# freiberg-roman/mj-grasp-sim

Hardware: NVIDIA B200
Metric: env_steps_per_s (higher is better)
Workload: dtype f32

## Files before the change

mj_grasp_sim_b200/csrc/mgs_common.cuh:

```cuda
#pragma once
#include <math.h>
#include <stdint.h>
#include <string.h>

#ifdef MGS_REAL_DOUBLE
typedef double real;
#define R_(x) x
#define REAL_EPS 2.2e-16
#else
typedef float real;
#define R_(x) x##f
#define REAL_EPS 1.2e-7f
#endif
#define MGS_MINVAL R_(1e-15)
#if !defined(MGS_REAL_DOUBLE) && !defined(MGS_NO_QPOS_COMP)
#define MGS_QPOS_COMP 1
#define MGS_NQ_LO(nq) (nq)
#else
#define MGS_NQ_LO(nq) 0
#endif

#ifdef MGS_HOST
#define MGS_DEV static inline
#define MGS_DEVN static
#define LANES 1
#define MGS_LANE 0
#define WSYNC() ((void)0)
#define LDG(p) (*(p))
#define MGS_STAGE_BARRIER(k) ((void)0)
#elif defined(MGS_WIDE)
#include <cuda_runtime.h>
#define MGS_DEV __device__ __forceinline__
#define MGS_DEVN static __device__ __noinline__
#define LANES MGS_WIDE
#define MGS_LANE ((int)threadIdx.x)
#define WSYNC() __syncthreads()
#define LDG(p) __ldg(p)
#define MGS_STAGE_BARRIER(k) ((void)0)
#else
#include <cuda_runtime.h>
#define MGS_DEV __device__ __forceinline__
#define MGS_DEVN static __device__ __noinline__
#define LANES 32
#define MGS_LANE ((int)(threadIdx.x & 31))
#define WSYNC() __syncwarp()
#define LDG(p) __ldg(p)
#ifndef MGS_BAR_MASK
#define MGS_BAR_MASK 63
#endif
#define MGS_STAGE_BARRIER(k) do { if ((MGS_BAR_MASK >> (k)) & 1) __syncthreads(); } while (0)
#endif

#ifndef MGS_INNER_UNROLL
#define MGS_INNER_UNROLL 4
#endif
#define MGS_PRAGMA_(x) _Pragma(#x)
#define MGS_PRAGMA(x) MGS_PRAGMA_(x)
#define MGS_UNROLL_INNER MGS_PRAGMA(unroll MGS_INNER_UNROLL)

#define PFOR(i, n) for (int i = MGS_LANE; i < (n); i += LANES)

enum { JNT_FREE = 0, JNT_BALL = 1, JNT_SLIDE = 2, JNT_HINGE = 3 };
enum { GEOM_SPHERE = 2, GEOM_CAPSULE = 3, GEOM_CYLINDER = 5, GEOM_BOX = 6, GEOM_MESH = 7 };
enum { EQ_CONNECT = 0, EQ_WELD = 1, EQ_JOINT = 2 };
enum { CT_EQUALITY = 0, CT_FRICTION_DOF = 1, CT_LIMIT = 2, CT_CONTACT = 3 };
enum { ST_SATISFIED = 0, ST_QUADRATIC = 1, ST_LINEARNEG = 2, ST_LINEARPOS = 3, ST_CONE = 4 };
enum { MGS_MODE_STEP = 0, MGS_MODE_COLLISION = 1, MGS_MODE_STABILITY = 2, MGS_MODE_CLUTTER_COLLISION = 3, MGS_MODE_CLUTTER_STABLE = 4 };

struct DevModel {
  int nq, nv, nu, nbody, njnt, neq, nmocap, ntendon, nwrap, ncgeom, npair, nhull;
  int maxdepth, max_tree_dofs, nM, ntree, ne_rows, nf_rows, ngravcomp, dofmask_words, cone_elliptic, iterations, ls_iterations, noslip_iterations, mpr_iterations, ground_geomid;
  real timestep, impratio, tolerance, ls_tolerance, noslip_tolerance, mpr_tolerance, meaninertia, gravity[3];
  const int *body_parentid, *body_rootid, *body_mocapid, *body_jntadr, *body_jntnum, *body_dofadr, *body_dofnum, *body_depth;
  const real *body_pos, *body_quat, *body_ipos, *body_iquat, *body_mass, *body_inertia, *body_invweight0, *body_subtreemass, *body_gravcomp;
  const int *jnt_type, *jnt_bodyid, *jnt_qposadr, *jnt_dofadr, *jnt_limited;
  const real *jnt_pos, *jnt_axis, *jnt_range, *jnt_stiffness, *jnt_solref, *jnt_solimp, *jnt_margin, *qpos0, *qpos_spring;
  const int *dof_bodyid, *dof_jntid, *dof_parentid, *dof_treeadr, *dof_treenum;
  const real *dof_armature, *dof_damping, *dof_frictionloss, *dof_solref, *dof_solimp, *dof_invweight0;
  const int *cgeom_geomid, *cgeom_type, *cgeom_bodyid, *cgeom_hullid;
  const real *cgeom_pos, *cgeom_quat, *cgeom_size, *cgeom_rbound;
  const int *hull_vertadr, *hull_vertnum, *hull_faceadr, *hull_facenum, *hull_facevertadr, *hull_facevertnum, *hull_facevert;
  const int *hull_nbradr, *hull_nbrnum, *hull_nbr;
  const real *hull_vert, *hull_facenormal;
  const int *pair_geom1, *pair_geom2, *pair_condim;
  const real *pair_friction, *pair_solref, *pair_solimp, *pair_margin;
  const int *tendon_adr, *tendon_num, *wrap_dofadr, *wrap_qposadr;
  const real *wrap_coef;
  const int *actuator_trntype, *actuator_trnid, *actuator_ctrllimited, *actuator_forcelimited;
  const real *actuator_gainprm, *actuator_biasprm, *actuator_ctrlrange, *actuator_forcerange, *actuator_gear;
  const int *eq_type, *eq_obj1id, *eq_obj2id, *eq_active, *eq_rowadr, *tri_ab;
  const int *dof_frictionrank;
  const int *dof_rowoff;
  const int *dof_blk;
  const int *blk_ij;
  const int *dof_treeid, *body_treeid;
  const int *tri_madr;
  const unsigned int *body_dofmask;
  const real *eq_data, *eq_solref, *eq_solimp;
  const real *mocap_pos0, *mocap_quat0;
};

#define MGS_LAYOUT_PERSIST(X)                                                                                      \
  X(hdr, 8) X(qpos, nq) X(qpos_lo, MGS_NQ_LO(nq)) X(qvel, nv) X(qacc_ws, nv) X(ctrl, nu) X(mocap, 7 * nmocap)                                          \
  X(xpos, 3 * nbody) X(xquat, 4 * nbody) X(xmat, 9 * nbody) X(rootcom, 3 * nbody) X(cdof, 6 * nv)                  \
  X(M, nM) X(Minv, nM) X(H, nv * nv)                                                                     \
  X(ten_length, ntendon) X(ten_J, ntendon * nv) X(act_moment, nu * nv) X(act_force, nu) X(act_length, nu)          \
  X(qfrc_smooth, nv) X(qacc_smooth, nv) X(qacc, nv) X(qfrc_constraint, nv) X(Ma, nv) X(grad, nv) X(search, nv)     \
  X(Mv, nv) X(wvec, nv) X(con_pos, 3 * ncon_max) X(con_normal, 3 * ncon_max) X(con_dist, ncon_max)                 \
  X(con_mu, ncon_max) X(con_pair, ncon_max) X(con_efc, ncon_max) X(nsB, 3 * nv) X(nsS, lanes + (lanes > 32 ? 8 : 0)) X(mpr_cache, 4 * ncache)
#define MGS_LAYOUT_TRANSIENT(X)                                                                                    \
  X(xipos, 3 * nbody) X(ximat, 9 * nbody) X(xanchor, 3 * njnt) X(xaxis, 3 * njnt) X(gxpos, 3 * ncgeom)             \
  X(gxmat, 9 * ncgeom) X(cinert, 10 * nbody) X(crb, 10 * nbody) X(cdof_dot, 6 * nv) X(cvel, 6 * nbody)             \
  X(cacc, 6 * nbody) X(cfrc, 6 * nbody)
#define MGS_LAYOUT_SOLVER(X)                                                                                       \
  X(J, nefc_max * nv) X(efc_D, nefc_max) X(efc_R, nefc_max) X(efc_aref, nefc_max) X(efc_aux, nefc_max)             \
  X(efc_force, nefc_max) X(efc_jar, nefc_max) X(efc_jv, nefc_max) X(efc_tsi, nefc_max)                                       \
  X(efc_key, (lanes > 32 ? nefc_max : 0)) X(efc_list, (lanes > 32 ? nefc_max : 0))
#define MGS_LAYOUT_FIELDS(X) MGS_LAYOUT_PERSIST(X) MGS_LAYOUT_TRANSIENT(X) MGS_LAYOUT_SOLVER(X)

struct Layout {
#define X(name, cnt) int name;
  MGS_LAYOUT_FIELDS(X)
#undef X
  int total, ncon_max, nefc_max, ncache;
  int req_off;
  int clip_off, nclip;
};

#define MGS_CLIP_STRIDE 109
#define MGS_MPR_CACHE_MAX 128
static inline void layout_compute(Layout *L, int nq, int nv, int nu, int nbody, int njnt, int nmocap, int ntendon, int ncgeom,
                                  int ncon_max, int nefc_max, int npair, int nM, int lanes = 32, int ncache_max = MGS_MPR_CACHE_MAX) {
  int off = 0;
  const int ncache = npair < ncache_max ? npair : ncache_max;
  L->ncache = ncache;
#define X(name, cnt) L->name = off; off += (cnt);
  MGS_LAYOUT_PERSIST(X)
  const int overlay = off;
  MGS_LAYOUT_TRANSIENT(X)
  const int end_t = off;
  off = overlay;
  MGS_LAYOUT_SOLVER(X)
#undef X
  L->total = off > end_t ? off : end_t;
  L->clip_off = end_t;
  L->nclip = (L->total - end_t) / MGS_CLIP_STRIDE;
  if (L->nclip < 1) { L->nclip = 1; L->total = end_t + MGS_CLIP_STRIDE; }
  if (L->nclip > 32) L->nclip = 32;
  L->req_off = L->clip_off + L->nclip * MGS_CLIP_STRIDE;
  if (lanes > 32 && L->total < L->req_off + 6 * lanes) L->total = L->req_off + 6 * lanes;
  L->total = (L->total + 3) & ~3;
  L->ncon_max = ncon_max;
  L->nefc_max = nefc_max;
}

#define MGS_MAX_NU 24
#define MGS_MAX_NJ 24
struct RolloutParams {
  int mode, n, nj, base_qposadr, nstep, nstep_close, nstep_lift, shake_steps, repose_on_close;
  real lift_dist, shake_dist;
  real qvel_clip;
  int joint_qposadr[MGS_MAX_NJ];
  real close_ctrl[MGS_MAX_NU];
};

struct BatchIO {
  const float *pose7;
  const float *joints;
  uint8_t *labels;
  int *steps;
  const real *state_in;
  real *state_out;
  real *diag_out;
  float *aux;
  int state_stride, diag_stride;
  unsigned int *work_counter;
  int *mpr_cache_g;
  real *env_state;
  const int *scene_index;
  int nscene;
  unsigned int *scene_success;
  int enough_stable;
};
```

mj_grasp_sim_b200/csrc/mgs_model_build.h:

```cpp
#pragma once
#include <string>
#include <vector>

#include "../../include/mgs_model_desc.h"
#include "mgs_common.cuh"

struct ModelBlob {
  std::vector<char> bytes;
  DevModel dm;
  int ncon_max, nefc_max;
  int rows_static, rows_per_contact;
  int nfreeobj;
};

namespace mgs_detail {
template <typename T, typename S>
inline const T *put(std::vector<char> &b, const S *src, size_t n) {
  size_t off = (b.size() + 15) & ~size_t(15);
  b.resize(off + (n ? n : 1) * sizeof(T));
  T *dst = reinterpret_cast<T *>(b.data() + off);
  for (size_t i = 0; i < n; i++) dst[i] = (T)src[i];
  return reinterpret_cast<const T *>(off);
}
}

inline bool build_model_blob(const MgsModelDesc *d, ModelBlob &out, std::string &err) {
  using mgs_detail::put;
  DevModel &m = out.dm;
  std::vector<char> &b = out.bytes;
  b.clear();
  b.resize(16);
  memset(&m, 0, sizeof(m));
  if (d->nu > MGS_MAX_NU) { err = "too many actuators"; return false; }
  if (d->nv > 255) { err = "nv > 255 (the lower-triangle index table packs a dof index in 8 bits)"; return false; }
  if (d->nmocap > 1) { err = "at most one mocap body is supported"; return false; }
  for (int p = 0; p < d->npair; p++)
    if (d->pair_condim[p] != 1 && d->pair_condim[p] != 3 && d->pair_condim[p] != 4) { err = "condim must be 1, 3 or 4"; return false; }
  for (int g = 0; g < d->ncgeom; g++) {
    int t = d->cgeom_type[g];
    if (t != GEOM_SPHERE && t != GEOM_CAPSULE && t != GEOM_CYLINDER && t != GEOM_BOX && t != GEOM_MESH) { err = "unsupported geom type"; return false; }
  }
  m.nq = d->nq; m.nv = d->nv; m.nu = d->nu; m.nbody = d->nbody; m.njnt = d->njnt; m.neq = d->neq; m.nmocap = d->nmocap;
  m.ntendon = d->ntendon; m.nwrap = d->nwrap; m.ncgeom = d->ncgeom; m.npair = d->npair; m.nhull = d->nhull;
  m.cone_elliptic = d->cone_elliptic; m.iterations = d->iterations; m.ls_iterations = d->ls_iterations;
  m.noslip_iterations = d->noslip_iterations; m.mpr_iterations = d->mpr_iterations; m.ground_geomid = d->ground_geomid;
  m.timestep = (real)d->timestep; m.impratio = (real)d->impratio; m.tolerance = (real)d->tolerance; m.ls_tolerance = (real)d->ls_tolerance;
  m.noslip_tolerance = (real)d->noslip_tolerance; m.mpr_tolerance = (real)d->mpr_tolerance; m.meaninertia = (real)d->meaninertia;
  for (int k = 0; k < 3; k++) m.gravity[k] = (real)d->gravity[k];
  const int nb = d->nbody, nv = d->nv, nq = d->nq, nj = d->njnt, nu = d->nu, ng = d->ncgeom, np = d->npair, nh = d->nhull;
  std::vector<int> depth(nb, 0), rowadr(d->neq, 0);
  std::vector<double> stm(nb, 0.0);
  int maxdepth = 0;
  for (int i = 1; i < nb; i++) { depth[i] = depth[d->body_parentid[i]] + 1; if (depth[i] > maxdepth) maxdepth = depth[i]; }
  for (int i = 0; i < nb; i++) stm[i] = d->body_mass[i];
  for (int i = nb - 1; i > 0; i--) stm[d->body_parentid[i]] += stm[i];
  int ne = 0;
  for (int q = 0; q < d->neq; q++) {
    rowadr[q] = ne;
    if (d->eq_active[q]) ne += d->eq_type[q] == EQ_WELD ? 6 : (d->eq_type[q] == EQ_CONNECT ? 3 : 1);
  }
  m.maxdepth = maxdepth; m.ne_rows = ne;
#define PI_(f, n) m.f = put<int>(b, d->f, (size_t)(n))
#define PR_(f, n) m.f = put<real>(b, d->f, (size_t)(n))
  PI_(body_parentid, nb); PI_(body_rootid, nb); PI_(body_mocapid, nb); PI_(body_jntadr, nb); PI_(body_jntnum, nb); PI_(body_dofadr, nb);
  PI_(body_dofnum, nb);
  m.body_depth = put<int>(b, depth.data(), nb);
  PR_(body_pos, 3 * nb); PR_(body_quat, 4 * nb); PR_(body_ipos, 3 * nb); PR_(body_iquat, 4 * nb); PR_(body_mass, nb); PR_(body_inertia, 3 * nb);
  PR_(body_invweight0, 2 * nb);
  m.body_subtreemass = put<real>(b, stm.data(), nb);
  PR_(body_gravcomp, nb);
  for (int i = 0; i < nb; i++) m.ngravcomp += (d->body_gravcomp[i] != 0 && d->body_mass[i] != 0);
  PI_(jnt_type, nj); PI_(jnt_bodyid, nj); PI_(jnt_qposadr, nj); PI_(jnt_dofadr, nj); PI_(jnt_limited, nj);
  PR_(jnt_pos, 3 * nj); PR_(jnt_axis, 3 * nj); PR_(jnt_range, 2 * nj); PR_(jnt_stiffness, nj); PR_(jnt_solref, 2 * nj); PR_(jnt_solimp, 5 * nj);
  PR_(jnt_margin, nj); PR_(qpos0, nq); PR_(qpos_spring, nq);
  PI_(dof_bodyid, nv); PI_(dof_jntid, nv); PI_(dof_parentid, nv);
  {
    std::vector<int> tadr(nv, 0), tnum(nv, 0);
    int maxt = 0;
    for (int i = 0; i < nv;) {
      int root = d->body_rootid[d->dof_bodyid[i]], j = i;
      while (j < nv && d->body_rootid[d->dof_bodyid[j]] == root) j++;
      for (int k = i; k < j; k++) { tadr[k] = i; tnum[k] = j - i; }
      if (j - i > maxt) maxt = j - i;
      i = j;
    }
    m.dof_treeadr = put<int>(b, tadr.data(), nv);
    m.dof_treenum = put<int>(b, tnum.data(), nv);
    m.max_tree_dofs = maxt;
    std::vector<int> rowoff(nv > 0 ? nv : 1, 0), ij;
    int nM = 0;
    for (int i = 0; i < nv;) {
      const int t = tnum[i];
      for (int r = 0; r < t; r++) {
        rowoff[i + r] = nM + r * t - i;
        for (int c = 0; c < t; c++) ij.push_back(((i + r) << 8) | (i + c));
      }
      nM += t * t;
      i += t;
    }
    m.nM = nM;
    std::vector<int> dtree(nv > 0 ? nv : 1, 0), btree(nb, -1);
    int ntree = 0;
    for (int i = 0; i < nv;) { for (int k = 0; k < tnum[i]; k++) dtree[i + k] = ntree; ntree++; i += tnum[i]; }
    for (int i = 1; i < nb; i++) {
      int bb = i;
      while (bb > 0 && d->body_dofnum[bb] == 0) bb = d->body_parentid[bb];
      if (bb > 0) btree[i] = dtree[d->body_dofadr[bb]];
    }
    m.ntree = ntree;
    m.dof_treeid = put<int>(b, dtree.data(), nv);
    m.body_treeid = put<int>(b, btree.data(), nb);
    m.dof_rowoff = put<int>(b, rowoff.data(), nv);
    std::vector<int> blkw(nv > 0 ? nv : 1, 0);
    for (int i = 0; i < nv; i++) blkw[i] = (int)((unsigned)rowoff[i] | ((unsigned)tadr[i] << 16) | ((unsigned)tnum[i] << 24));
    m.dof_blk = put<int>(b, blkw.data(), nv);
    m.blk_ij = put<int>(b, ij.data(), ij.size());
    std::vector<int> tm;
    for (int a = 0; a < nv; a++)
      for (int c = 0; c <= a; c++) tm.push_back(tadr[a] == tadr[c] ? rowoff[a] + c : -1);
    m.tri_madr = put<int>(b, tm.data(), tm.size());
  }
  PR_(dof_armature, nv); PR_(dof_damping, nv); PR_(dof_frictionloss, nv); PR_(dof_solref, 2 * nv); PR_(dof_solimp, 5 * nv); PR_(dof_invweight0, nv);
  PI_(cgeom_geomid, ng); PI_(cgeom_type, ng); PI_(cgeom_bodyid, ng); PI_(cgeom_hullid, ng);
  PR_(cgeom_pos, 3 * ng); PR_(cgeom_quat, 4 * ng); PR_(cgeom_size, 3 * ng); PR_(cgeom_rbound, ng);
  PI_(hull_vertadr, nh); PI_(hull_vertnum, nh); PI_(hull_faceadr, nh); PI_(hull_facenum, nh); PI_(hull_facevertadr, d->nhullface);
  PI_(hull_facevertnum, d->nhullface); PI_(hull_facevert, d->nhullfacevert); PI_(hull_nbradr, d->nhullvert); PI_(hull_nbrnum, d->nhullvert);
  PI_(hull_nbr, d->nhullnbr); PR_(hull_vert, 3 * d->nhullvert); PR_(hull_facenormal, 3 * d->nhullface);
  PI_(pair_geom1, np); PI_(pair_geom2, np); PI_(pair_condim, np); PR_(pair_friction, 5 * np); PR_(pair_solref, 2 * np); PR_(pair_solimp, 5 * np);
  PR_(pair_margin, np);
  PI_(tendon_adr, d->ntendon); PI_(tendon_num, d->ntendon); PI_(wrap_dofadr, d->nwrap); PI_(wrap_qposadr, d->nwrap); PR_(wrap_coef, d->nwrap);
  PI_(actuator_trntype, nu); PI_(actuator_trnid, nu); PI_(actuator_ctrllimited, nu); PI_(actuator_forcelimited, nu);
  PR_(actuator_gainprm, 3 * nu); PR_(actuator_biasprm, 3 * nu); PR_(actuator_ctrlrange, 2 * nu); PR_(actuator_forcerange, 2 * nu); PR_(actuator_gear, nu);
  PI_(eq_type, d->neq); PI_(eq_obj1id, d->neq); PI_(eq_obj2id, d->neq); PI_(eq_active, d->neq);
  m.eq_rowadr = put<int>(b, rowadr.data(), d->neq);
  std::vector<int> tri;
  for (int a = 0; a < nv; a++)
    for (int c = 0; c <= a; c++) tri.push_back((a << 8) | c);
  m.tri_ab = put<int>(b, tri.data(), tri.size());
  {
    std::vector<int> rank(nv > 0 ? nv : 1, -1);
    int nfr_rows = 0;
    for (int i = 0; i < nv; i++) if (d->dof_frictionloss[i] > 0) rank[i] = nfr_rows++;
    m.nf_rows = nfr_rows;
    m.dof_frictionrank = put<int>(b, rank.data(), nv);
  }
  {
    const int words = (nv + 31) / 32 > 0 ? (nv + 31) / 32 : 1;
    std::vector<unsigned int> mask((size_t)nb * words, 0u);
    for (int i = 1; i < nb; i++) {
      int bb = i;
      while (bb > 0 && d->body_dofnum[bb] == 0) bb = d->body_parentid[bb];
      if (bb == 0) continue;
      for (int k = d->body_dofadr[bb] + d->body_dofnum[bb] - 1; k >= 0; k = d->dof_parentid[k]) mask[(size_t)i * words + (k >> 5)] |= 1u << (k & 31);
    }
    m.dofmask_words = words;
    m.body_dofmask = put<unsigned int>(b, mask.data(), mask.size());
  }
  PR_(eq_data, 11 * d->neq); PR_(eq_solref, 2 * d->neq); PR_(eq_solimp, 5 * d->neq);
  PR_(mocap_pos0, 3 * d->nmocap); PR_(mocap_quat0, 4 * d->nmocap);
#undef PI_
#undef PR_
  int nfr = 0, nlim = 0;
  for (int i = 0; i < nv; i++) nfr += d->dof_frictionloss[i] > 0;
  for (int j = 0; j < nj; j++) nlim += d->jnt_limited[j] ? 1 : 0;
  int maxdim = 1;
  for (int p = 0; p < np; p++) if (d->pair_condim[p] > maxdim) maxdim = d->pair_condim[p];
  int nobjpair = 0;
  for (int p = 0; p < np; p++) {
    for (int side = 0; side < 2; side++) {
      const int bd = d->cgeom_bodyid[side ? d->pair_geom2[p] : d->pair_geom1[p]];
      bool leaf = true;
      for (int c = 0; c < nb; c++) if (d->body_parentid[c] == bd && c != bd) leaf = false;
      if (d->body_parentid[bd] == 0 && d->body_dofnum[bd] == 6 && leaf) { nobjpair++; break; }
    }
  }
  int nc = 2 * nobjpair;
  nc = nc < 32 ? 32 : (nc > 64 ? 64 : nc);
  int nfreeobj = 0;
  for (int bd = 1; bd < nb; bd++) {
    bool leaf = true;
    for (int c = 0; c < nb; c++) if (d->body_parentid[c] == bd && c != bd) leaf = false;
    if (d->body_parentid[bd] == 0 && d->body_dofnum[bd] == 6 && leaf && d->body_mocapid[bd] < 0) nfreeobj++;
  }
  if (nv > 24 && nfreeobj <= 1) nc = 32;
  nc = (nc + 3) & ~3;
  out.ncon_max = nc;
  out.nfreeobj = nfreeobj;
  out.rows_static = ne + nfr + nlim;
  out.rows_per_contact = maxdim < 3 ? 3 : maxdim;
  out.nefc_max = out.rows_static + nc * out.rows_per_contact;
  return true;
}

inline void rebase_model(DevModel &m, const char *base) {
  const char **p = reinterpret_cast<const char **>(&m.body_parentid);
  const char **end = reinterpret_cast<const char **>(&m.mocap_quat0) + 1;
  for (; p != end; ++p) *p = base + reinterpret_cast<size_t>(*p);
}
```

mj_grasp_sim_b200/csrc/mgs_sim.cuh:

```cuda
#pragma once
#include "mgs_common.cuh"

#ifdef MGS_HOST
MGS_DEV real wsum(real x) { return x; }
MGS_DEV int wsumi(int x) { return x; }
MGS_DEV int wany(int p) { return p; }
MGS_DEV int wscan_excl(int x, int *total) { *total = x; return 0; }
MGS_DEV real wbcast(real x, int src) { (void)src; return x; }
MGS_DEV int wbcasti(int x, int src) { (void)src; return x; }
MGS_DEV void wargmax(real &v, int &idx) { (void)v; (void)idx; }
MGS_DEV int wrank(int p, int *total) { *total = p ? 1 : 0; return 0; }
MGS_DEV int wfirst(int p) { return p ? 0 : -1; }
MGS_DEV void wsum3(real &a, real &b, real &c) { (void)a; (void)b; (void)c; }
#elif defined(MGS_WIDE)
#define MGS_NWARP (MGS_WIDE / 32)
static __shared__ real mgs_cta_r[3 * MGS_NWARP];
static __shared__ int mgs_cta_i[MGS_NWARP];
MGS_DEV void wsum3(real &a, real &b, real &c) {
#pragma unroll
  for (int o = 16; o > 0; o >>= 1) {
    a += __shfl_xor_sync(0xffffffffu, a, o); b += __shfl_xor_sync(0xffffffffu, b, o); c += __shfl_xor_sync(0xffffffffu, c, o);
  }
  if ((threadIdx.x & 31) == 0) { mgs_cta_r[threadIdx.x >> 5] = a; mgs_cta_r[MGS_NWARP + (threadIdx.x >> 5)] = b; mgs_cta_r[2 * MGS_NWARP + (threadIdx.x >> 5)] = c; }
  __syncthreads();
// ... 432 lines not shown
      for (int k = k0; k < kk; k++) xi -= L[ro + (k - i) * s + i] * x[k];
    }
  }
  WSYNC();
}
#else
MGS_DEVN void chol_factor_w(real *A, int n, int blocked, real *colbuf = (real *)0) {
  const int nsteps = blocked ? MD.max_tree_dofs : n;
  if (LANES == 32 && n <= LANES) {
    const int i = MGS_LANE;
    int tadr = 0, tnum = n, ro = i * n, s = n;
    if (i < n) row_addr(i, n, blocked, ro, s, tadr, tnum);
    WSYNC();
    #pragma unroll 1
    for (int t = 0; t < nsteps; t++) {
      const int j = tadr + t;
      const int live = (i < n) && (t < tnum);
      real d = 1, lij = 0;
      if (live) {
        d = A[ro + (j - i) * s + j];
        d = sqrt(d > MGS_MINVAL ? d : MGS_MINVAL);
        if (i > j) { lij = A[ro + j] * (R_(1.0) / d); A[ro + j] = lij; }
      }
      WSYNC();
      if (live) {
        if (i == j) A[ro + j] = d;
        else if (i > j) {
          const real *col = A + ro + (j + 1 - i) * s + j;
          real *row = A + ro + j + 1;
          const int cnt = i - j;
          MGS_UNROLL_INNER
          for (int k = 0; k < cnt; k++) row[k] -= lij * col[k * s];
        }
      }
      WSYNC();
    }
    WSYNC();
    return;
  }
  #pragma unroll 1
  for (int t = 0; t < nsteps; t++) {
    WSYNC();
    #pragma unroll 1
    PFOR(i, n) {
      int ro, s, tadr, tnum;
      row_addr(i, n, blocked, ro, s, tadr, tnum);
      if (i == tadr + t) { const real d = A[ro + i]; A[ro + i] = sqrt(d > MGS_MINVAL ? d : MGS_MINVAL); }
    }
    WSYNC();
    #pragma unroll 1
    PFOR(i, n) {
      int ro, s, tadr, tnum;
      row_addr(i, n, blocked, ro, s, tadr, tnum);
      const int j = tadr + t;
      if (t < tnum && i > j) A[ro + j] /= A[ro + (j - i) * s + j];
    }
    WSYNC();
    #pragma unroll 1
    PFOR(i, n) {
      int ro, s, tadr, tnum;
      row_addr(i, n, blocked, ro, s, tadr, tnum);
      const int j = tadr + t;
      if (t < tnum && i > j) {
        const real lij = A[ro + j];
        const real *col = A + ro + (j + 1 - i) * s + j;
        real *row = A + ro + j + 1;
        const int cnt = i - j;
        MGS_UNROLL_INNER
        for (int k = 0; k < cnt; k++) row[k] -= lij * col[k * s];
      }
    }
  }
  WSYNC();
}
MGS_DEVN void chol_solve_w(const real *L, real *x, int n, int blocked) {
  const int nsteps = blocked ? MD.max_tree_dofs : n;
  if (LANES == 32 && n <= LANES) {
    const int i = MGS_LANE;
    int tadr = 0, tnum = n, ro = i * n, s = n;
    if (i < n) row_addr(i, n, blocked, ro, s, tadr, tnum);
    WSYNC();
    real xi = (i < n) ? x[i] : R_(0.0);
    #pragma unroll 1
    for (int t = 0; t < nsteps; t++) {
      const int k = tadr + t, live = (i < n) && (t < tnum);
      const real xs = __shfl_sync(0xffffffffu, xi, live ? k : i);
      if (live) {
        const real xk = xs / L[ro + (k - i) * s + k];
        if (i == k) xi = xk;
        else if (i > k) xi -= L[ro + k] * xk;
      }
    }
    #pragma unroll 1
    for (int t = nsteps - 1; t >= 0; t--) {
      const int k = tadr + t, live = (i < n) && (t < tnum);
      const real xs = __shfl_sync(0xffffffffu, xi, live ? k : i);
      if (live) {
        const real xk = xs / L[ro + (k - i) * s + k];
        if (i == k) xi = xk;
        else if (i < k) xi -= L[ro + (k - i) * s + i] * xk;
      }
    }
    if (i < n) x[i] = xi;
    WSYNC();
    return;
  }
  #pragma unroll 1
  for (int pass = 0; pass < 2; pass++) {
    #pragma unroll 1
    for (int tt = 0; tt < nsteps; tt++) {
      const int t = pass == 0 ? tt : nsteps - 1 - tt;
      WSYNC();
      #pragma unroll 1
      PFOR(i, n) {
        int ro, s, tadr, tnum;
        row_addr(i, n, blocked, ro, s, tadr, tnum);
        if (i == tadr + t) x[i] /= L[ro + i];
      }
      WSYNC();
      #pragma unroll 1
      PFOR(i, n) {
        int ro, s, tadr, tnum;
        row_addr(i, n, blocked, ro, s, tadr, tnum);
        const int k = tadr + t;
        if (t >= tnum) continue;
        if (pass == 0 && i > k) x[i] -= L[ro + k] * x[k];
        else if (pass == 1 && i < k) x[i] -= L[ro + (k - i) * s + i] * x[k];
      }
    }
  }
  WSYNC();
}
#endif
MGS_DEVN void chol_inverse_w(const real *L, real *Ainv, int n) {
  #pragma unroll 1
  PFOR(c, n) {
    int roc, lo, t;
    blk_row(c, roc, lo, t);
    const int bo = roc - (c - lo) * t + lo;
    const real *Lt = L + bo;
    real *At = Ainv + bo;
    const int cl = c - lo;
    #pragma unroll 1
    for (int i = 0; i < t; i++) {
      real sacc = (i == cl) ? R_(1.0) : R_(0.0);
      MGS_UNROLL_INNER
      for (int k = 0; k < i; k++) sacc -= Lt[i * t + k] * At[k * t + cl];
      At[i * t + cl] = sacc / Lt[i * t + i];
    }
    #pragma unroll 1
    for (int i = t - 1; i >= 0; i--) {
      real sacc = At[i * t + cl];
      MGS_UNROLL_INNER
      for (int k = i + 1; k < t; k++) sacc -= Lt[k * t + i] * At[k * t + cl];
      At[i * t + cl] = sacc / Lt[i * t + i];
    }
  }
  WSYNC();
}
MGS_DEVN void matvec_w(real *y, const real *A, const real *x, int n) {
  #pragma unroll 1
  PFOR(i, n) {
    int ro, lo, tn;
    blk_row(i, ro, lo, tn);
    const int hi = lo + tn;
    const real *row = A + ro;
    real t = 0;
    MGS_UNROLL_INNER
    for (int j = lo; j < hi; j++) t += row[j] * x[j];
    y[i] = t;
  }
  WSYNC();
}

MGS_DEVN void kinematics_w(Env &e) {
  #pragma unroll 1
  PFOR(i, 1) {
    EF(xpos)[0] = EF(xpos)[1] = EF(xpos)[2] = 0;
    EF(xquat)[0] = 1; EF(xquat)[1] = EF(xquat)[2] = EF(xquat)[3] = 0;
    for (int k = 0; k < 9; k++) EF(xmat)[k] = EF(ximat)[k] = (k % 4 == 0) ? R_(1.0) : R_(0.0);
    EF(xipos)[0] = EF(xipos)[1] = EF(xipos)[2] = 0;
  }
  WSYNC();
  #pragma unroll 1
  for (int lvl = 1; lvl <= MD.maxdepth; lvl++) {
    #pragma unroll 1
    PFOR(b, MD.nbody) {
      if (LDG(MD.body_depth + b) != lvl) continue;
      int p = LDG(MD.body_parentid + b);
      real xp[3], xq[4], t[3], bq[4];
      int mid = LDG(MD.body_mocapid + b);
      if (mid >= 0) {
        copy3(xp, EF(mocap) + 7 * mid);
        xq[0] = EF(mocap)[7 * mid + 3]; xq[1] = EF(mocap)[7 * mid + 4]; xq[2] = EF(mocap)[7 * mid + 5]; xq[3] = EF(mocap)[7 * mid + 6];
        normquat(xq);
      } else {
        ld3(t, MD.body_pos + 3 * b);
        mulmatvec3(xp, EF(xmat) + 9 * p, t);
        add3(xp, xp, EF(xpos) + 3 * p);
        ld4(bq, MD.body_quat + 4 * b);
        mulquat(xq, EF(xquat) + 4 * p, bq);
      }
      int ja = LDG(MD.body_jntadr + b), jn = LDG(MD.body_jntnum + b);
      #pragma unroll 1
      for (int j = ja; j < ja + jn; j++) {
        int qa = LDG(MD.jnt_qposadr + j), jt = LDG(MD.jnt_type + j);
        real *anchor = EF(xanchor) + 3 * j, *axis = EF(xaxis) + 3 * j;
        if (jt == JNT_FREE) {
          copy3(xp, EF(qpos) + qa);
#ifdef MGS_QPOS_COMP
          xq[0] = EF(qpos)[qa + 3]; xq[1] = EF(qpos)[qa + 4]; xq[2] = EF(qpos)[qa + 5]; xq[3] = EF(qpos)[qa + 6];
          if (fabs(xq[0] * xq[0] + xq[1] * xq[1] + xq[2] * xq[2] + xq[3] * xq[3] - R_(1.0)) > R_(1e-5)) {
            normquat(EF(qpos) + qa + 3);
            for (int k = 3; k < 7; k++) { xq[k - 3] = EF(qpos)[qa + k]; QPOS_LO_CLEAR(qa + k); }
          } else normquat(xq);
#else
          normquat(EF(qpos) + qa + 3);
          xq[0] = EF(qpos)[qa + 3]; xq[1] = EF(qpos)[qa + 4]; xq[2] = EF(qpos)[qa + 5]; xq[3] = EF(qpos)[qa + 6];
#endif
          copy3(anchor, xp);
          axis[0] = 0; axis[1] = 0; axis[2] = 1;
          continue;
        }
        real Rm[9], ja3[3], jp3[3];
        quat2mat(Rm, xq);
        ld3(ja3, MD.jnt_axis + 3 * j); ld3(jp3, MD.jnt_pos + 3 * j);
        mulmatvec3(axis, Rm, ja3);
        mulmatvec3(anchor, Rm, jp3);
        add3(anchor, anchor, xp);
        real dq = EF(qpos)[qa] - LDG(MD.qpos0 + qa);
        if (jt == JNT_SLIDE) {
          addscl3(xp, axis, dq);
        } else {
          real sn = sin(R_(0.5) * dq), cs = cos(R_(0.5) * dq);
          real ql[4] = {cs, sn * ja3[0], sn * ja3[1], sn * ja3[2]};
          mulquat(xq, xq, ql);
          quat2mat(Rm, xq);
          mulmatvec3(t, Rm, jp3);
          sub3(xp, anchor, t);
        }
      }
      normquat(xq);
      copy3(EF(xpos) + 3 * b, xp);
      EF(xquat)[4 * b] = xq[0]; EF(xquat)[4 * b + 1] = xq[1]; EF(xquat)[4 * b + 2] = xq[2]; EF(xquat)[4 * b + 3] = xq[3];
      quat2mat(EF(xmat) + 9 * b, xq);
      ld3(t, MD.body_ipos + 3 * b);
      mulmatvec3(t, EF(xmat) + 9 * b, t);
      add3(EF(xipos) + 3 * b, xp, t);
      ld4(bq, MD.body_iquat + 4 * b);
      real qi[4];
      mulquat(qi, xq, bq);
      quat2mat(EF(ximat) + 9 * b, qi);
    }
    WSYNC();
  }
  #pragma unroll 1
  PFOR(g, MD.ncgeom) {
    int b = LDG(MD.cgeom_bodyid + g);
    real t[3], q[4], gq[4];
    ld3(t, MD.cgeom_pos + 3 * g);
    mulmatvec3(t, EF(xmat) + 9 * b, t);
    add3(EF(gxpos) + 3 * g, EF(xpos) + 3 * b, t);
    ld4(gq, MD.cgeom_quat + 4 * g);
    mulquat(q, EF(xquat) + 4 * b, gq);
    quat2mat(EF(gxmat) + 9 * g, q);
  }
  WSYNC();
}

MGS_DEV void mul_inert_vec(real *res, const real *I, const real *v) {
  real t[3];
  res[0] = I[0] * v[0] + I[3] * v[1] + I[4] * v[2];
  res[1] = I[3] * v[0] + I[1] * v[1] + I[5] * v[2];
  res[2] = I[4] * v[0] + I[5] * v[1] + I[2] * v[2];
  cross3(t, I + 6, v + 3);
  add3(res, res, t);
  cross3(t, I + 6, v);
  res[3] = I[9] * v[3] - t[0]; res[4] = I[9] * v[4] - t[1]; res[5] = I[9] * v[5] - t[2];
}
MGS_DEV void cross_motion(real *res, const real *vel, const real *v) {
  real t[3];
  cross3(res, vel, v);
  cross3(res + 3, vel, v + 3);
  cross3(t, vel + 3, v);
  add3(res + 3, res + 3, t);
}
MGS_DEV void cross_force(real *res, const real *vel, const real *f) {
  real t[3];
  cross3(res, vel, f);
  cross3(t, vel + 3, f + 3);
  add3(res, res, t);
  cross3(res + 3, vel, f + 3);
}

MGS_DEVN void inertia_w(Env &e) {
  const int nb = MD.nbody, nv = MD.nv;
  #pragma unroll 1
  PFOR(b, nb) {
    if (b == 0 || LDG(MD.body_parentid + b) != 0) continue;
    real c[3] = {0, 0, 0}, mt = LDG(MD.body_subtreemass + b);
    if (mt < MGS_MINVAL) copy3(c, EF(xipos) + 3 * b);
    else {
      #pragma unroll 1
      for (int k = b; k < nb; k++)
        if (LDG(MD.body_rootid + k) == b) addscl3(c, EF(xipos) + 3 * k, LDG(MD.body_mass + k));
      scl3(c, c, R_(1.0) / mt);
    }
    copy3(EF(rootcom) + 3 * b, c);
  }
  WSYNC();
  #pragma unroll 1
  PFOR(b, nb) {
    real *ci = EF(cinert) + 10 * b;
    if (b == 0) { for (int k = 0; k < 10; k++) ci[k] = 0; continue; }
    real dif[3], diag[3], mass = LDG(MD.body_mass + b);
    const real *Rm = EF(ximat) + 9 * b;
    sub3(dif, EF(xipos) + 3 * b, EF(rootcom) + 3 * LDG(MD.body_rootid + b));
    ld3(diag, MD.body_inertia + 3 * b);
    real I[6];
    I[0] = Rm[0] * diag[0] * Rm[0] + Rm[1] * diag[1] * Rm[1] + Rm[2] * diag[2] * Rm[2];
    I[1] = Rm[3] * diag[0] * Rm[3] + Rm[4] * diag[1] * Rm[4] + Rm[5] * diag[2] * Rm[5];
    I[2] = Rm[6] * diag[0] * Rm[6] + Rm[7] * diag[1] * Rm[7] + Rm[8] * diag[2] * Rm[8];
    I[3] = Rm[0] * diag[0] * Rm[3] + Rm[1] * diag[1] * Rm[4] + Rm[2] * diag[2] * Rm[5];
    I[4] = Rm[0] * diag[0] * Rm[6] + Rm[1] * diag[1] * Rm[7] + Rm[2] * diag[2] * Rm[8];
    I[5] = Rm[3] * diag[0] * Rm[6] + Rm[4] * diag[1] * Rm[7] + Rm[5] * diag[2] * Rm[8];
    real d2 = dot3(dif, dif);
    ci[0] = I[0] + mass * (d2 - dif[0] * dif[0]);
    ci[1] = I[1] + mass * (d2 - dif[1] * dif[1]);
    ci[2] = I[2] + mass * (d2 - dif[2] * dif[2]);
    ci[3] = I[3] - mass * dif[0] * dif[1];
    ci[4] = I[4] - mass * dif[0] * dif[2];
    ci[5] = I[5] - mass * dif[1] * dif[2];
    ci[6] = mass * dif[0]; ci[7] = mass * dif[1]; ci[8] = mass * dif[2]; ci[9] = mass;
    for (int k = 0; k < 10; k++) EF(crb)[10 * b + k] = ci[k];
  }
  #pragma unroll 1
  PFOR(j, MD.njnt) {
    int b = LDG(MD.jnt_bodyid + j), da = LDG(MD.jnt_dofadr + j), jt = LDG(MD.jnt_type + j);
    real off[3];
    sub3(off, EF(rootcom) + 3 * LDG(MD.body_rootid + b), EF(xanchor) + 3 * j);
    if (jt == JNT_FREE) {
      for (int k = 0; k < 36; k++) EF(cdof)[6 * da + k] = 0;
      for (int k = 0; k < 3; k++) EF(cdof)[6 * (da + k) + 3 + k] = 1;
      for (int k = 0; k < 3; k++) {
        real ax[3] = {EF(xmat)[9 * b + k], EF(xmat)[9 * b + 3 + k], EF(xmat)[9 * b + 6 + k]};
        real *c = EF(cdof) + 6 * (da + 3 + k);
        copy3(c, ax);
        cross3(c + 3, ax, off);
      }
    } else if (jt == JNT_SLIDE) {
      real *c = EF(cdof) + 6 * da;
      c[0] = c[1] = c[2] = 0;
      copy3(c + 3, EF(xaxis) + 3 * j);
    } else {
      real *c = EF(cdof) + 6 * da;
      copy3(c, EF(xaxis) + 3 * j);
      cross3(c + 3, EF(xaxis) + 3 * j, off);
    }
  }
  #pragma unroll 1
  PFOR(i, MD.nM) EF(M)[i] = 0;
  WSYNC();
  #pragma unroll 1
  for (int lvl = MD.maxdepth - 1; lvl >= 1; lvl--) {
    #pragma unroll 1
    PFOR(b, nb) {
      if (LDG(MD.body_depth + b) != lvl) continue;
      #pragma unroll 1
      for (int c = b + 1; c < nb; c++)
        if (LDG(MD.body_parentid + c) == b)
          for (int k = 0; k < 10; k++) EF(crb)[10 * b + k] += EF(crb)[10 * c + k];
    }
    WSYNC();
  }
  #pragma unroll 1
  PFOR(i, nv) {
    real buf[6];
    mul_inert_vec(buf, EF(crb) + 10 * LDG(MD.dof_bodyid + i), EF(cdof) + 6 * i);
    #pragma unroll 1
    for (int j = i; j >= 0; j = LDG(MD.dof_parentid + j)) {
      real v = 0;
      for (int k = 0; k < 6; k++) v += EF(cdof)[6 * j + k] * buf[k];
      if (j == i) v += LDG(MD.dof_armature + i);
      EF(M)[LDG(MD.dof_rowoff + i) + j] = v;
      EF(M)[LDG(MD.dof_rowoff + j) + i] = v;
    }
  }
  WSYNC();
  #pragma unroll 1
  PFOR(i, MD.nM) EF(H)[i] = EF(M)[i];
  chol_factor_w(EF(H), nv, 1);
  chol_inverse_w(EF(H), EF(Minv), nv);
}

MGS_DEVN void transmission_w(Env &e) {
  const int nv = MD.nv;
  #pragma unroll 1
  PFOR(i, MD.ntendon * nv) EF(ten_J)[i] = 0;
  #pragma unroll 1
  PFOR(i, MD.nu * nv) EF(act_moment)[i] = 0;
  WSYNC();
  #pragma unroll 1
  PFOR(t, MD.ntendon) {
    real L = 0;
    int a = LDG(MD.tendon_adr + t), n = LDG(MD.tendon_num + t);
    #pragma unroll 1
    for (int w = a; w < a + n; w++) {
      real c = LDG(MD.wrap_coef + w);
      L += c * EF(qpos)[LDG(MD.wrap_qposadr + w)];
      EF(ten_J)[t * nv + LDG(MD.wrap_dofadr + w)] += c;
    }
    EF(ten_length)[t] = L;
  }
  WSYNC();
  #pragma unroll 1
  PFOR(a, MD.nu) {
    real gear = LDG(MD.actuator_gear + a);
    int id = LDG(MD.actuator_trnid + a);
    if (LDG(MD.actuator_trntype + a) == 0) {
      EF(act_length)[a] = gear * EF(qpos)[LDG(MD.jnt_qposadr + id)];
      EF(act_moment)[a * nv + LDG(MD.jnt_dofadr + id)] = gear;
    } else {
      EF(act_length)[a] = gear * EF(ten_length)[id];
      #pragma unroll 1
      for (int d = 0; d < nv; d++) EF(act_moment)[a * nv + d] = gear * EF(ten_J)[id * nv + d];
    }
  }
  WSYNC();
}

MGS_DEVN void smooth_forces_w(Env &e) {
  const int nb = MD.nbody, nv = MD.nv;
  #pragma unroll 1
  PFOR(k, 6) { EF(cvel)[k] = 0; EF(cfrc)[k] = 0; EF(cacc)[k] = (k < 3) ? R_(0.0) : -MD.gravity[k - 3]; }
  WSYNC();
  #pragma unroll 1
  for (int lvl = 1; lvl <= MD.maxdepth; lvl++) {
    #pragma unroll 1
    PFOR(b, nb) {
      if (LDG(MD.body_depth + b) != lvl) continue;
      int p = LDG(MD.body_parentid + b);
      real cv[6], ca[6];
      for (int k = 0; k < 6; k++) { cv[k] = EF(cvel)[6 * p + k]; ca[k] = EF(cacc)[6 * p + k]; }
      int ja = LDG(MD.body_jntadr + b), jn = LDG(MD.body_jntnum + b);
      #pragma unroll 1
      for (int j = ja; j < ja + jn; j++) {
        int da = LDG(MD.jnt_dofadr + j);
        if (LDG(MD.jnt_type + j) == JNT_FREE) {
          for (int k = 0; k < 18; k++) EF(cdof_dot)[6 * da + k] = 0;
          for (int k = 0; k < 3; k++)
            for (int c = 0; c < 6; c++) cv[c] += EF(cdof)[6 * (da + k) + c] * EF(qvel)[da + k];
          for (int k = 3; k < 6; k++) cross_motion(EF(cdof_dot) + 6 * (da + k), cv, EF(cdof) + 6 * (da + k));
          for (int k = 3; k < 6; k++)
            for (int c = 0; c < 6; c++) cv[c] += EF(cdof)[6 * (da + k) + c] * EF(qvel)[da + k];
          for (int k = 3; k < 6; k++)
            for (int c = 0; c < 6; c++) ca[c] += EF(cdof_dot)[6 * (da + k) + c] * EF(qvel)[da + k];
        } else {
          cross_motion(EF(cdof_dot) + 6 * da, cv, EF(cdof) + 6 * da);
          for (int c = 0; c < 6; c++) { cv[c] += EF(cdof)[6 * da + c] * EF(qvel)[da]; ca[c] += EF(cdof_dot)[6 * da + c] * EF(qvel)[da]; }
        }
      }
      real t1[6], t2[6];
      mul_inert_vec(t1, EF(cinert) + 10 * b, cv);
      cross_force(t2, cv, t1);
      mul_inert_vec(t1, EF(cinert) + 10 * b, ca);
      for (int k = 0; k < 6; k++) { EF(cvel)[6 * b + k] = cv[k]; EF(cacc)[6 * b + k] = ca[k]; EF(cfrc)[6 * b + k] = t1[k] + t2[k]; }
    }
    WSYNC();
  }
  #pragma unroll 1
  for (int lvl = MD.maxdepth - 1; lvl >= 1; lvl--) {
    #pragma unroll 1
    PFOR(b, nb) {
      if (LDG(MD.body_depth + b) != lvl) continue;
      #pragma unroll 1
      for (int c = b + 1; c < nb; c++)
        if (LDG(MD.body_parentid + c) == b)
          for (int k = 0; k < 6; k++) EF(cfrc)[6 * b + k] += EF(cfrc)[6 * c + k];
    }
    WSYNC();
  }
  #pragma unroll 1
  PFOR(a, MD.nu) {
    real c = EF(ctrl)[a], vel = 0;
    if (LDG(MD.actuator_ctrllimited + a)) c = fmax(LDG(MD.actuator_ctrlrange + 2 * a), fmin(LDG(MD.actuator_ctrlrange + 2 * a + 1), c));
    #pragma unroll 1
    for (int d = 0; d < nv; d++) vel += EF(act_moment)[a * nv + d] * EF(qvel)[d];
    real f = LDG(MD.actuator_gainprm + 3 * a) * c + LDG(MD.actuator_biasprm + 3 * a) + LDG(MD.actuator_biasprm + 3 * a + 1) * EF(act_length)[a] +
             LDG(MD.actuator_biasprm + 3 * a + 2) * vel;
    if (LDG(MD.actuator_forcelimited + a)) f = fmax(LDG(MD.actuator_forcerange + 2 * a), fmin(LDG(MD.actuator_forcerange + 2 * a + 1), f));
    EF(act_force)[a] = f;
  }
  WSYNC();
  #pragma unroll 1
  PFOR(d, nv) {
    real bias = 0;
    int b = LDG(MD.dof_bodyid + d);
    for (int c = 0; c < 6; c++) bias += EF(cdof)[6 * d + c] * EF(cfrc)[6 * b + c];
    real f = -LDG(MD.dof_damping + d) * EF(qvel)[d] - bias;
    int j = LDG(MD.dof_jntid + d);
    if (LDG(MD.jnt_type + j) != JNT_FREE) {
      real k = LDG(MD.jnt_stiffness + j);
      int qa = LDG(MD.jnt_qposadr + j);
      if (k != 0) f -= k * (EF(qpos)[qa] - LDG(MD.qpos_spring + qa));
    }
    #pragma unroll 1
    for (int a = 0; a < MD.nu; a++) f += EF(act_moment)[a * nv + d] * EF(act_force)[a];
    EF(qfrc_smooth)[d] = f;
  }
  WSYNC();
  if (MD.ngravcomp > 0) {
    #pragma unroll 1
    PFOR(one, 1) {
      #pragma unroll 1
      for (int b = 1; b < nb; b++) {
        const real gc = LDG(MD.body_gravcomp + b), mass = LDG(MD.body_mass + b);
        if (gc == 0 || mass == 0) continue;
        real off[3], f[3] = {-MD.gravity[0] * mass * gc, -MD.gravity[1] * mass * gc, -MD.gravity[2] * mass * gc};
        off[0] = EF(cinert)[10 * b + 6] / mass; off[1] = EF(cinert)[10 * b + 7] / mass; off[2] = EF(cinert)[10 * b + 8] / mass;
        int bb = b;
        while (bb > 0 && LDG(MD.body_dofnum + bb) == 0) bb = LDG(MD.body_parentid + bb);
        if (bb == 0) continue;
        #pragma unroll 1
        for (int d = LDG(MD.body_dofadr + bb) + LDG(MD.body_dofnum + bb) - 1; d >= 0; d = LDG(MD.dof_parentid + d)) {
          const real *c = EF(cdof) + 6 * d;
          real lin[3];
          cross3(lin, c, off);
          EF(qfrc_smooth)[d] += (lin[0] + c[3]) * f[0] + (lin[1] + c[4]) * f[1] + (lin[2] + c[5]) * f[2];
        }
      }
    }
    WSYNC();
  }
  matvec_w(EF(qacc_smooth), EF(Minv), EF(qfrc_smooth), nv);
}
```

Before: 4.993 million.

## Precompute per-level body lists and child/subtree adjacency for tree passes

Builds CSR-style arrays on the host for bodies grouped by depth, the children of each body, and the bodies in each root subtree, then stores them in the device model. The forward and backward tree sweeps in COM, CRB and bias-force computation now iterate only over the bodies at the current level and their actual children, instead of scanning all bodies and testing depth or parent on each pass. The body-force computation (inertia times acceleration plus the velocity cross term) is moved out of the level loop into one pass over all bodies, which improves lane utilisation. The cost is extra indirect loads and a larger model struct whose rebase range now has to include the new pointers.

```diff
diff --git a/mj_grasp_sim_b200/csrc/mgs_common.cuh b/mj_grasp_sim_b200/csrc/mgs_common.cuh
--- a/mj_grasp_sim_b200/csrc/mgs_common.cuh
+++ b/mj_grasp_sim_b200/csrc/mgs_common.cuh
@@ -59,6 +59,7 @@
 #define MGS_UNROLL_INNER MGS_PRAGMA(unroll MGS_INNER_UNROLL)
 
 #define PFOR(i, n) for (int i = MGS_LANE; i < (n); i += LANES)
+#define PFOR_RANGE(i, a, b) for (int i = (a) + MGS_LANE; i < (b); i += LANES)
 
 enum { JNT_FREE = 0, JNT_BALL = 1, JNT_SLIDE = 2, JNT_HINGE = 3 };
 enum { GEOM_SPHERE = 2, GEOM_CAPSULE = 3, GEOM_CYLINDER = 5, GEOM_BOX = 6, GEOM_MESH = 7 };
@@ -98,6 +99,9 @@
   const unsigned int *body_dofmask;
   const real *eq_data, *eq_solref, *eq_solimp;
   const real *mocap_pos0, *mocap_quat0;
+  const int *level_adr, *level_body;
+  const int *child_adr, *child_body;
+  const int *tree_adr, *tree_body;
 };
 
 #define MGS_LAYOUT_PERSIST(X)                                                                                      \
diff --git a/mj_grasp_sim_b200/csrc/mgs_model_build.h b/mj_grasp_sim_b200/csrc/mgs_model_build.h
--- a/mj_grasp_sim_b200/csrc/mgs_model_build.h
+++ b/mj_grasp_sim_b200/csrc/mgs_model_build.h
@@ -160,6 +160,19 @@
   PR_(mocap_pos0, 3 * d->nmocap); PR_(mocap_quat0, 4 * d->nmocap);
 #undef PI_
 #undef PR_
+  {
+    std::vector<int> ladr(maxdepth + 2, 0), lbody(nb), cadr(nb + 1, 0), cbody(nb > 1 ? nb - 1 : 1), tadr(nb + 1, 0), tbody(nb > 1 ? nb - 1 : 1);
+    for (int i = 0; i < nb; i++) ladr[depth[i] + 1]++;
+    for (int i = 1; i < nb; i++) { cadr[d->body_parentid[i] + 1]++; tadr[d->body_rootid[i] + 1]++; }
+    for (int l = 0; l <= maxdepth; l++) ladr[l + 1] += ladr[l];
+    for (int i = 0; i < nb; i++) { cadr[i + 1] += cadr[i]; tadr[i + 1] += tadr[i]; }
+    std::vector<int> lf(ladr.begin(), ladr.end() - 1), cf(cadr.begin(), cadr.end() - 1), tf(tadr.begin(), tadr.end() - 1);
+    for (int i = 0; i < nb; i++) lbody[lf[depth[i]]++] = i;
+    for (int i = 1; i < nb; i++) { cbody[cf[d->body_parentid[i]]++] = i; tbody[tf[d->body_rootid[i]]++] = i; }
+    m.level_adr = put<int>(b, ladr.data(), ladr.size()); m.level_body = put<int>(b, lbody.data(), nb);
+    m.child_adr = put<int>(b, cadr.data(), cadr.size()); m.child_body = put<int>(b, cbody.data(), nb - 1);
+    m.tree_adr = put<int>(b, tadr.data(), tadr.size()); m.tree_body = put<int>(b, tbody.data(), nb - 1);
+  }
   int nfr = 0, nlim = 0;
   for (int i = 0; i < nv; i++) nfr += d->dof_frictionloss[i] > 0;
   for (int j = 0; j < nj; j++) nlim += d->jnt_limited[j] ? 1 : 0;
@@ -194,6 +207,6 @@
 
 inline void rebase_model(DevModel &m, const char *base) {
   const char **p = reinterpret_cast<const char **>(&m.body_parentid);
-  const char **end = reinterpret_cast<const char **>(&m.mocap_quat0) + 1;
+  const char **end = reinterpret_cast<const char **>(&m.tree_body) + 1;
   for (; p != end; ++p) *p = base + reinterpret_cast<size_t>(*p);
 }
diff --git a/mj_grasp_sim_b200/csrc/mgs_sim.cuh b/mj_grasp_sim_b200/csrc/mgs_sim.cuh
--- a/mj_grasp_sim_b200/csrc/mgs_sim.cuh
+++ b/mj_grasp_sim_b200/csrc/mgs_sim.cuh
@@ -758,8 +758,10 @@
     if (mt < MGS_MINVAL) copy3(c, EF(xipos) + 3 * b);
     else {
       #pragma unroll 1
-      for (int k = b; k < nb; k++)
-        if (LDG(MD.body_rootid + k) == b) addscl3(c, EF(xipos) + 3 * k, LDG(MD.body_mass + k));
+      for (int i = LDG(MD.tree_adr + b), ie = LDG(MD.tree_adr + b + 1); i < ie; i++) {
+        const int k = LDG(MD.tree_body + i);
+        addscl3(c, EF(xipos) + 3 * k, LDG(MD.body_mass + k));
+      }
       scl3(c, c, R_(1.0) / mt);
     }
     copy3(EF(rootcom) + 3 * b, c);
@@ -819,13 +821,15 @@
   WSYNC();
   #pragma unroll 1
   for (int lvl = MD.maxdepth - 1; lvl >= 1; lvl--) {
-    #pragma unroll 1
-    PFOR(b, nb) {
-      if (LDG(MD.body_depth + b) != lvl) continue;
-      #pragma unroll 1
-      for (int c = b + 1; c < nb; c++)
-        if (LDG(MD.body_parentid + c) == b)
-          for (int k = 0; k < 10; k++) EF(crb)[10 * b + k] += EF(crb)[10 * c + k];
+    const int l1 = LDG(MD.level_adr + lvl + 1);
+    #pragma unroll 1
+    PFOR_RANGE(i, LDG(MD.level_adr + lvl), l1) {
+      const int b = LDG(MD.level_body + i);
+      #pragma unroll 1
+      for (int q = LDG(MD.child_adr + b), qe = LDG(MD.child_adr + b + 1); q < qe; q++) {
+        const int c = LDG(MD.child_body + q);
+        for (int k = 0; k < 10; k++) EF(crb)[10 * b + k] += EF(crb)[10 * c + k];
+      }
     }
     WSYNC();
   }
@@ -892,9 +896,10 @@
   WSYNC();
   #pragma unroll 1
   for (int lvl = 1; lvl <= MD.maxdepth; lvl++) {
-    #pragma unroll 1
-    PFOR(b, nb) {
-      if (LDG(MD.body_depth + b) != lvl) continue;
+    const int l1 = LDG(MD.level_adr + lvl + 1);
+    #pragma unroll 1
+    PFOR_RANGE(i, LDG(MD.level_adr + lvl), l1) {
+      const int b = LDG(MD.level_body + i);
       int p = LDG(MD.body_parentid + b);
       real cv[6], ca[6];
       for (int k = 0; k < 6; k++) { cv[k] = EF(cvel)[6 * p + k]; ca[k] = EF(cacc)[6 * p + k]; }
@@ -916,23 +921,32 @@
           for (int c = 0; c < 6; c++) { cv[c] += EF(cdof)[6 * da + c] * EF(qvel)[da]; ca[c] += EF(cdof_dot)[6 * da + c] * EF(qvel)[da]; }
         }
       }
-      real t1[6], t2[6];
-      mul_inert_vec(t1, EF(cinert) + 10 * b, cv);
-      cross_force(t2, cv, t1);
-      mul_inert_vec(t1, EF(cinert) + 10 * b, ca);
-      for (int k = 0; k < 6; k++) { EF(cvel)[6 * b + k] = cv[k]; EF(cacc)[6 * b + k] = ca[k]; EF(cfrc)[6 * b + k] = t1[k] + t2[k]; }
-    }
-    WSYNC();
-  }
+      for (int k = 0; k < 6; k++) { EF(cvel)[6 * b + k] = cv[k]; EF(cacc)[6 * b + k] = ca[k]; }
+    }
+    WSYNC();
+  }
+  #pragma unroll 1
+  PFOR(i, nb - 1) {
+    const int b = i + 1;
+    real t1[6], t2[6];
+    const real *cv = EF(cvel) + 6 * b;
+    mul_inert_vec(t1, EF(cinert) + 10 * b, cv);
+    cross_force(t2, cv, t1);
+    mul_inert_vec(t1, EF(cinert) + 10 * b, EF(cacc) + 6 * b);
+    for (int k = 0; k < 6; k++) EF(cfrc)[6 * b + k] = t1[k] + t2[k];
+  }
+  WSYNC();
   #pragma unroll 1
   for (int lvl = MD.maxdepth - 1; lvl >= 1; lvl--) {
-    #pragma unroll 1
-    PFOR(b, nb) {
-      if (LDG(MD.body_depth + b) != lvl) continue;
-      #pragma unroll 1
-      for (int c = b + 1; c < nb; c++)
-        if (LDG(MD.body_parentid + c) == b)
-          for (int k = 0; k < 6; k++) EF(cfrc)[6 * b + k] += EF(cfrc)[6 * c + k];
+    const int l1 = LDG(MD.level_adr + lvl + 1);
+    #pragma unroll 1
+    PFOR_RANGE(i, LDG(MD.level_adr + lvl), l1) {
+      const int b = LDG(MD.level_body + i);
+      #pragma unroll 1
+      for (int q = LDG(MD.child_adr + b), qe = LDG(MD.child_adr + b + 1); q < qe; q++) {
+        const int c = LDG(MD.child_body + q);
+        for (int k = 0; k < 6; k++) EF(cfrc)[6 * b + k] += EF(cfrc)[6 * c + k];
+      }
     }
     WSYNC();
   }
```

Measured after the change: 5.110 million, median of 6. +2.3%, better.
